# jsdjayanga/kmer-counter

Measured on NVIDIA B200. Metric: k-mers counted/s at k=31, higher is better.
Workload: dtype u64

## Files before the change

### kmer-counter_b200/csrc/kc_super.cu

```cuda
#include <math.h>
#include <stdlib.h>

#include "kc_internal.h"
#include "kc_super.cuh"

namespace kc {

namespace {

constexpr uint32_t kNoBin = 0xffffffffu;
constexpr int kSwThreads = 256;
constexpr int kSwMaxSeg = 18;
constexpr int kNb1Max = 1024;
constexpr int kRsBins = 2048;

template <uint32_t X> struct ILog2 { static constexpr uint32_t v = 1 + ILog2<(X >> 1)>::v; };
template <> struct ILog2<1> { static constexpr uint32_t v = 0; };

__host__ __device__ __forceinline__ uint32_t mmer_hash(uint32_t mm) {
    uint32_t h = mm * 0x9E3779B1u;
    h ^= h >> 15;
    h *= 0x85EBCA6Bu;
    return h;
}
// ... 1003 lines not shown
    if (total) owner = (uint32_t)((bk_lo + (bk_hi - bk_lo) / 2) * P / total);
    if (owner >= P) owner = P - 1;
    atomicMin(&s_lo[owner], bk0);
    __syncthreads();
    if (tid == 0) {
        s_lo[P] = NB;
        for (int o = (int)P - 1; o >= 0; o--)
            if (s_lo[o] > s_lo[o + 1]) s_lo[o] = s_lo[o + 1];
        s_lo[0] = 0;
        if (keep_ranges)
            for (uint32_t o = 0; o <= P; o++) s_lo[o] = x->lo[o];
        for (uint32_t o = 0; o <= P; o++) x->lo[o] = s_lo[o];
        uint32_t widest = 1;
        for (uint32_t o = 0; o < P; o++) {
            const uint32_t wd = ((s_lo[o + 1] + (1u << fold) - 1) >> fold) - (s_lo[o] >> fold);
            widest = wd > widest ? wd : widest;
        }
        while (s_b2 > 0 && ((unsigned long long)widest << s_b2) > kSuperMaxSub) s_b2--;
        s_large = (large_plan || (total >> (b1 + s_b2)) > sub_target) ? 1 : 0;
    }
    __syncthreads();
    const uint32_t my_lo = s_lo[rank], my_hi = s_lo[rank + 1];
    unsigned long long n_recv = 0;
    for (uint32_t s2 = 0; s2 < P; s2++) {
        const unsigned long long incl = block_incl(all_hist[s2 * NB + tid]);
        if (tid == 0) { s_b = 0; s_e = 0; }
        __syncthreads();
        if (my_lo > 0 && tid == (int)my_lo - 1) s_b = incl;
        if (my_hi > 0 && tid == (int)my_hi - 1) s_e = incl;
        __syncthreads();
        if (tid == 0) { x->src_range[s2][0] = (uint32_t)s_b; x->src_range[s2][1] = (uint32_t)s_e; }
        n_recv += s_e - s_b;
        __syncthreads();
    }
    {
        const uint32_t nb1 = 1u << b1;
        uint32_t c = 0;
        if ((uint32_t)tid < nb1)
            for (int j = 0; j < (1 << fold); j++) c += all_hist[rank * NB + ((uint32_t)tid << fold) + j];
        const unsigned long long incl = block_incl(c);
        if ((uint32_t)tid < nb1) {
            base1[tid] = (uint32_t)(incl - c);
            cursor1[tid] = (uint32_t)(incl - c);
            if ((uint32_t)tid == nb1 - 1) base1[nb1] = (uint32_t)incl;
        }
    }
    if (tid == 0) {
        const int b2 = s_b2;
        unsigned long long nd = sc[SW_D];
        if (nd > d_cap) nd = d_cap;
        uint32_t any_ovf = 0;
        for (uint32_t s2 = 0; s2 < P; s2++)
            if (peers.sc[s2][SW_OVF] != 0) any_ovf = 1;
        plan->n_d = (uint32_t)nd;
        plan->b1 = (uint32_t)b1;
        plan->b2 = (uint32_t)b2;
        plan->shift2 = 64 - b1 - b2;
        plan->sub0 = (my_lo >> fold) << b2;
        plan->n_sub = (((my_hi + (1u << fold) - 1) >> fold) << b2) - plan->sub0;
        plan->prefix_bits = b1 + b2;
        x->n_recv = (uint32_t)(n_recv > 0xffffffffull ? 0xffffffffull : n_recv);
        x->any_ovf = any_ovf;
        x->fin_large = (uint32_t)s_large;
        if (n_recv > d_cap) atomicOr(&sc[SW_FAIL], 16ull);
    }
}

struct XPeers {
    const uint64_t *keys[8];
    const uint32_t *counts[8];
    const uint32_t *hist2[8];
};
__global__ void __launch_bounds__(256) x_merge_hist_kernel(XPeers peers, uint32_t P, const SuperPlanDev *__restrict__ plan,
                                                           uint32_t *__restrict__ out) {
    const uint32_t n = plan->n_sub, sub0 = plan->sub0;
    for (uint32_t j = blockIdx.x * blockDim.x + threadIdx.x; j < n; j += gridDim.x * blockDim.x) {
        uint32_t c = 0;
        for (uint32_t s2 = 0; s2 < P; s2++) c += peers.hist2[s2][sub0 + j];
        out[j] = c;
    }
}

constexpr int kRsThreads = 256;
template <int W> struct RsCfg { static constexpr int ITEMS = 16 / W, TILE = kRsThreads * ITEMS; };

template <int W, int LEVEL>
__global__ void __launch_bounds__(kRsThreads) rec_scatter_kernel(const uint64_t *__restrict__ in_keys,
                                                                 const uint32_t *__restrict__ in_counts,
                                                                 uint64_t *__restrict__ out_keys,
                                                                 uint32_t *__restrict__ out_counts,
                                                                 const SuperPlanDev *__restrict__ plan, int b1,
                                                                 const unsigned long long *__restrict__ n_ptr, uint64_t cap,
                                                                 uint32_t *__restrict__ g_cursor,
                                                                 const uint32_t *__restrict__ range) {
    constexpr int ITEMS = RsCfg<W>::ITEMS, TILE = RsCfg<W>::TILE;
    extern __shared__ __align__(16) uint8_t rs_smem[];
    Key<W> *stg_k = reinterpret_cast<Key<W> *>(rs_smem);
    uint32_t *stg_c = reinterpret_cast<uint32_t *>(stg_k + TILE);
    uint32_t *cnt = stg_c + TILE, *start = cnt + kRsBinsPadded, *gbase = start + kRsBinsPadded;
    __shared__ uint32_t s_warp[kRsThreads / 32];
    uint32_t n, first = 0;
    if (LEVEL == 1) {
        unsigned long long nn = *n_ptr;
        n = (uint32_t)(nn > cap ? cap : nn);
    } else if (range) {
        first = range[0];
        n = range[1];
    } else {
        n = plan->n_d;
    }
    const int b2 = LEVEL == 1 ? 0 : (int)plan->b2;
    if (LEVEL == 1) b1 = (int)plan->b1;
    const int shift = LEVEL == 1 ? 64 - b1 : (int)plan->shift2;
    const uint32_t nb2 = 1u << b2;
    const uint32_t sub0 = LEVEL == 1 ? 0u : plan->sub0;
    for (uint32_t begin = first + blockIdx.x * (uint32_t)TILE; begin < n; begin += gridDim.x * (uint32_t)TILE) {
        const uint32_t end = begin + TILE < n ? begin + TILE : n;
        Key<W> key[ITEMS];
        uint32_t val[ITEMS];
        uint16_t rank[ITEMS];
#pragma unroll
        for (int i = 0; i < ITEMS; i++) {
            const uint32_t idx = begin + i * kRsThreads + threadIdx.x;
            if (idx < end) { key[i] = ld_key<W>(in_keys, idx); val[i] = in_counts[idx]; }
            else { key[i].w[0] = 0; val[i] = 0; }
        }
        uint32_t p0 = 0, nb;
        if (LEVEL == 1) {
            nb = 1u << b1;
        } else {
            p0 = ((uint32_t)(in_keys[(size_t)begin * W] >> shift) >> b2) << b2;
            const uint32_t pl = (uint32_t)(in_keys[(size_t)(end - 1) * W] >> shift);
            nb = (pl >> b2) == (p0 >> b2) || 2 * nb2 > (uint32_t)kRsBins ? nb2 : 2 * nb2;
        }
        for (uint32_t i = threadIdx.x; i < nb; i += kRsThreads) cnt[pad32(i)] = 0;
        __syncthreads();
#pragma unroll
        for (int i = 0; i < ITEMS; i++) {
            const uint32_t idx = begin + i * kRsThreads + threadIdx.x;
            rank[i] = 0xffffu;
            if (idx < end) {
                const uint32_t pfx = (uint32_t)(key[i].w[0] >> shift);
                const uint32_t rel = pfx - p0;
                if (rel < nb) rank[i] = (uint16_t)atomicAdd(&cnt[pad32(rel)], 1u);
                else {
                    const uint32_t o = atomicAdd(&g_cursor[pfx - sub0], 1u);
                    st_key<W>(out_keys, o, key[i]);
                    out_counts[o] = val[i];
                }
            }
        }
        __syncthreads();
        const uint32_t total = block_scan_bins<kRsThreads>(cnt, start, (int)nb, s_warp);
        uint32_t reserved[kRsBins / kRsThreads];
#pragma unroll
        for (int u = 0; u < kRsBins / kRsThreads; u++) {
            const uint32_t b = u * kRsThreads + threadIdx.x;
            reserved[u] = 0;
            if (b < nb) {
                const uint32_t c = cnt[pad32(b)];
                if (c) reserved[u] = atomicAdd(&g_cursor[p0 - sub0 + b], c);
            }
        }
#pragma unroll
        for (int i = 0; i < ITEMS; i++)
            if (rank[i] != 0xffffu) {
                const uint32_t o = start[pad32((uint32_t)(key[i].w[0] >> shift) - p0)] + rank[i];
                stg_k[o] = key[i];
                stg_c[o] = val[i];
            }
#pragma unroll
        for (int u = 0; u < kRsBins / kRsThreads; u++) {
            const uint32_t b = u * kRsThreads + threadIdx.x;
            if (b < nb) gbase[pad32(b)] = reserved[u] - start[pad32(b)];
        }
        __syncthreads();
        for (uint32_t i = threadIdx.x; i < total; i += kRsThreads) {
            const Key<W> k = stg_k[i];
            const uint32_t o = gbase[pad32((uint32_t)(k.w[0] >> shift) - p0)] + i;
            st_key<W>(out_keys, o, k);
            out_counts[o] = stg_c[i];
        }
        __syncthreads();
    }
}

template <int W>
__global__ void __launch_bounds__(256) place_init_kernel(const uint64_t *__restrict__ keys, uint32_t *__restrict__ counts,
                                                         uint64_t n, int shift1, uint32_t *__restrict__ hist1,
                                                         unsigned long long *__restrict__ sc) {
    __shared__ uint32_t sh[kNb1Max];
    for (uint32_t i = threadIdx.x; i < kNb1Max; i += 256) sh[i] = 0;
    __syncthreads();
    for (uint64_t i = blockIdx.x * 256ull + threadIdx.x; i < n; i += gridDim.x * 256ull) {
        counts[i] = 1u;
        atomicAdd(&sh[(uint32_t)(keys[i * W] >> shift1)], 1u);
    }
    __syncthreads();
    for (uint32_t i = threadIdx.x; i < kNb1Max; i += 256) {
        const uint32_t c = sh[i];
        if (c) atomicAdd(&hist1[i], c);
    }
    if (blockIdx.x == 0 && threadIdx.x == 0) sc[SW_D] = n;
}

template <int W>
__global__ void place_fix_zero_kernel(const uint64_t *__restrict__ keys, uint32_t *__restrict__ counts,
                                      const unsigned long long *__restrict__ n_invalid) {
    bool zero = true;
    for (int w = 0; w < W; w++) zero = zero && keys[w] == 0;
    if (zero) counts[0] -= (uint32_t)*n_invalid;
}

constexpr uint32_t kH2Chunk = 16384;
template <int W>
__global__ void __launch_bounds__(256) rec_hist2_kernel(const uint64_t *__restrict__ keys,
                                                        const SuperPlanDev *__restrict__ plan,
                                                        uint32_t *__restrict__ g_hist2) {
    __shared__ uint32_t sh[kRsBins];
    const uint32_t n = plan->n_d;
    const int b2 = (int)plan->b2, shift2 = (int)plan->shift2;
    const uint32_t nb2 = 1u << b2, m2 = nb2 - 1;
    for (uint32_t begin = blockIdx.x * kH2Chunk; begin < n; begin += gridDim.x * kH2Chunk) {
        const uint32_t end = begin + kH2Chunk < n ? begin + kH2Chunk : n;
        for (uint32_t i = threadIdx.x; i < nb2; i += 256) sh[i] = 0;
        const uint32_t b0 = (uint32_t)(keys[(size_t)begin * W] >> shift2) >> b2;
        __syncthreads();
#pragma unroll 4
        for (uint32_t i = begin + threadIdx.x; i < end; i += 256) {
            const uint32_t pfx = (uint32_t)(keys[(size_t)i * W] >> shift2);
            if ((pfx >> b2) == b0) atomicAdd(&sh[pfx & m2], 1u);
            else atomicAdd(&g_hist2[pfx], 1u);
        }
        __syncthreads();
        for (uint32_t i = threadIdx.x; i < nb2; i += 256) {
            const uint32_t c = sh[i];
            if (c) atomicAdd(&g_hist2[(size_t)b0 * nb2 + i], c);
        }
        __syncthreads();
    }
}

constexpr uint32_t kScanTile = 4096;
__global__ void __launch_bounds__(1024) sw_scan_kernel(const uint32_t *__restrict__ hist, const uint32_t *__restrict__ n_ptr,
                                                       uint32_t n_host, uint32_t *__restrict__ base,
                                                       uint32_t *__restrict__ cursor, unsigned long long *total_out) {
    __shared__ uint32_t s_w[32];
    __shared__ uint32_t s_carry;
    const uint32_t n = n_ptr ? *n_ptr : n_host;
    const uint32_t tid = threadIdx.x, lane = tid & 31, warp = tid >> 5;
    const uint32_t t0 = blockIdx.x * kScanTile;
    if (t0 >= n) return;
    uint32_t acc = 0;
#pragma unroll 8
    for (uint32_t i = tid; i < t0; i += 1024) acc += hist[i];
#pragma unroll
    for (int o = 16; o > 0; o >>= 1) acc += __shfl_xor_sync(0xffffffffu, acc, o);
    if (lane == 0) s_w[warp] = acc;
    __syncthreads();
    if (tid == 0) {
        uint32_t c = 0;
        for (int w = 0; w < 32; w++) c += s_w[w];
        s_carry = c;
    }
    __syncthreads();
    const uint32_t i0 = t0 + tid * 4;
    uint32_t v[4];
#pragma unroll
    for (int u = 0; u < 4; u++) v[u] = i0 + u < n ? hist[i0 + u] : 0;
    const uint32_t sum = v[0] + v[1] + v[2] + v[3];
    uint32_t incl = sum;
#pragma unroll
    for (int o = 1; o < 32; o <<= 1) {
        uint32_t t = __shfl_up_sync(0xffffffffu, incl, o);
        if (lane >= (uint32_t)o) incl += t;
    }
    __syncthreads();
    if (lane == 31) s_w[warp] = incl;
    __syncthreads();
    uint32_t off = s_carry, tot = 0;
#pragma unroll
    for (uint32_t w = 0; w < 32; w++) {
        const uint32_t x = s_w[w];
        if (w < warp) off += x;
        tot += x;
    }
    uint32_t run = off + incl - sum;
#pragma unroll
    for (int u = 0; u < 4; u++) {
        if (i0 + u < n) { base[i0 + u] = run; if (cursor) cursor[i0 + u] = run; }
        run += v[u];
    }
    if (tid == 0 && t0 + kScanTile >= n) {
        base[n] = s_carry + tot;
        if (total_out) *total_out = s_carry + tot;
    }
}

__device__ __forceinline__ uint32_t pow2_ceil_u32(uint32_t x) { return x <= 1 ? 1u : 1u << (32 - __clz(x - 1)); }

struct FinishParams {
    const uint64_t *in_keys;
    const uint32_t *in_counts;
    const uint32_t *base2;
    const SuperPlanDev *plan;
    uint64_t *out_keys;
    uint32_t *out_counts;
    uint32_t *m_out;
    uint32_t *big;
    unsigned long long *sc;
};

template <int W, int THREADS, int CAP, bool DUP>
__global__ void __launch_bounds__(THREADS) rec_finish_kernel(FinishParams p) {
    constexpr int kPer = CAP / THREADS;
    extern __shared__ __align__(16) uint8_t fs_smem[];
    Key<W> *sk = reinterpret_cast<Key<W> *>(fs_smem);
    Key<W> *fk = sk + (DUP ? CAP : 0);
    uint32_t *scn = reinterpret_cast<uint32_t *>(fk + CAP);
    uint32_t *fc = scn + (DUP ? CAP : 0);
    uint32_t *c3 = fc + CAP;
    uint32_t *s3 = c3 + CAP + CAP / 32;
    __shared__ uint32_t s_maxbin, s_cnt, s_j, s_b, s_e;
    __shared__ uint32_t s_warp[THREADS / 32];
    const uint32_t tid = threadIdx.x, lane = tid & 31, warp = tid >> 5;
    const uint32_t n_sub = p.plan->n_sub;
    const int prefix_bits = (int)p.plan->prefix_bits;
    unsigned long long folded_local = 0;
    uint32_t t1 = 0, t2 = 0, b1 = 0, e1 = 0;
    if (tid == 0) {
        t1 = (uint32_t)atomicAdd(&p.sc[SW_TICKET2], 1ull);
        t2 = t1 < n_sub ? (uint32_t)atomicAdd(&p.sc[SW_TICKET2], 1ull) : n_sub;
        if (t1 < n_sub) { b1 = p.base2[t1]; e1 = p.base2[t1 + 1]; }
    }

    while (true) {
        if (tid == 0) {
            s_j = t1; s_b = b1; s_e = e1;
            t1 = t2;
            if (t1 < n_sub) {
                b1 = p.base2[t1]; e1 = p.base2[t1 + 1];
                t2 = (uint32_t)atomicAdd(&p.sc[SW_TICKET2], 1ull);
            }
        }
        __syncthreads();
        const uint32_t j = s_j;
        if (j >= n_sub) break;
        const uint32_t b = s_b, n = s_e - b;
        if (n == 0) {
            if (tid == 0) { p.big[j] = 0; if (DUP) p.m_out[j] = 0; }
            __syncthreads();
            continue;
        }
        if (n > (uint32_t)CAP) {
            if (tid == 0) {
                p.big[j] = n;
                atomicAdd(&p.sc[SW_BIG], 1ull);
                atomicAdd(&p.sc[SW_BIG_RECORDS], (unsigned long long)n);
                if (DUP) p.m_out[j] = 0;
            }
            __syncthreads();
            continue;
        }
        if (tid == 0) p.big[j] = 0;
        Key<W> rk[kPer];
        uint32_t rc[kPer], rr[kPer];
#pragma unroll
        for (int u = 0; u < kPer; u++) {
            const uint32_t i = u * THREADS + tid;
            if (u * THREADS >= n) break;
            if (i < n) { rk[u] = ld_key<W>(p.in_keys, b + i); rc[u] = p.in_counts[b + i]; }
        }
        uint32_t nb3 = 2 * pow2_ceil_u32(n);
        nb3 = nb3 < 64 ? 64 : (nb3 > (uint32_t)CAP ? (uint32_t)CAP : nb3);
        int shift3 = 64 - prefix_bits - (31 - __clz(nb3));
        if (shift3 < 0) shift3 = 0;
        for (uint32_t i = tid; i < nb3; i += THREADS) c3[pad32(i)] = 0;
        if (tid == 0) { s_maxbin = 0; s_cnt = 0; }
        __syncthreads();
#pragma unroll
        for (int u = 0; u < kPer; u++) {
            const uint32_t i = u * THREADS + tid;
            if (u * THREADS >= n) break;
            if (i < n) rr[u] = atomicAdd(&c3[pad32((uint32_t)(rk[u].w[0] >> shift3) & (nb3 - 1))], 1u);
        }
        __syncthreads();
        {
            const uint32_t per3 = nb3 >= (uint32_t)THREADS ? nb3 / THREADS : 1u;
            const uint32_t b0 = tid * per3;
            uint32_t sum = 0, mx = 0;
            if (b0 < nb3)
                for (uint32_t q = 0; q < per3; q++) { const uint32_t v = c3[pad32(b0 + q)]; sum += v; mx = max(mx, v); }
            if (mx > 2) atomicMax(&s_maxbin, mx);
            uint32_t incl = sum;
#pragma unroll
            for (int o = 1; o < 32; o <<= 1) {
                uint32_t t = __shfl_up_sync(0xffffffffu, incl, o);
// ... 408 lines not shown
cudaError_t super_scatter(const SuperPlan &pl, const void *d_reads, uint64_t n_reads, void *ws,
                          unsigned long long *d_sc, int n_sms, cudaStream_t s) {
    if (pl.W == 1) return super_scatter_w<1>(pl, d_reads, n_reads, ws, d_sc, n_sms, s);
    if (pl.W == 2) return super_scatter_w<2>(pl, d_reads, n_reads, ws, d_sc, n_sms, s);
    return cudaErrorInvalidValue;
}

template <int W, int THREADS, int TSLOTS, int RPT = 2, bool CANON = false>
static cudaError_t launch_count(const SwCountParams &cp, int n_sms, cudaStream_t s) {
    const uint32_t RB = THREADS * RPT, RT = W == 1 ? (RPT > 1 ? RB : 2 * RB) : 1;
    const uint32_t smem = TSLOTS * (8 * W + 4) + RB * 16 * W + THREADS * 4 + kNb1Max * 4 +
                          (THREADS / 32) * (RPT > 1 ? 64 : 96) * (8 * W + 4) + RT * 20 + RB * 4 + 64;
    auto kern = sw_count_kernel<W, THREADS, TSLOTS, RPT, CANON>;
    cudaError_t e = cudaFuncSetAttribute(kern, cudaFuncAttributeMaxDynamicSharedMemorySize, (int)smem);
    if (e != cudaSuccess) return e;
    int per_sm = 1;
    cudaOccupancyMaxActiveBlocksPerMultiprocessor(&per_sm, kern, THREADS, smem);
    if (per_sm < 1) per_sm = 1;
    kern<<<(uint32_t)n_sms * per_sm, THREADS, smem, s>>>(cp);
    return cudaGetLastError();
}

template <int W>
static cudaError_t super_count_bins_w(const SuperPlan &pl, bool add_phantom, void *ws, unsigned long long *d_sc, int n_sms,
                                      cudaStream_t s, void *const *peer_ws = nullptr, uint32_t rank = 0,
                                      uint32_t n_ranks = 1) {
    cudaError_t e;
    SwCountParams cp{};
    const uint32_t n_src = peer_ws ? n_ranks : 1u;
    cp.n_src = n_src;
    for (uint32_t i = 0; i < n_src; i++) {
        void *w = peer_ws ? peer_ws[i] : ws;
        cp.src_cursor[i] = at<uint32_t>(w, pl.off_cursor);
        cp.src_bins[i] = at<uint8_t>(w, pl.off_bins);
        cp.src_sc[i] = peer_ws ? at<unsigned long long>(w, pl.off_sc) : d_sc;
    }
    cp.bin_begin = peer_ws ? (uint32_t)((uint64_t)pl.n_bins * rank / n_ranks) : 0u;
    cp.n_bins = peer_ws ? (uint32_t)((uint64_t)pl.n_bins * (rank + 1) / n_ranks) - cp.bin_begin : pl.n_bins;
    cp.ovf = at<uint8_t>(ws, pl.off_ovf);
    cp.bin_cap = pl.bin_cap; cp.ovf_slice = pl.ovf_slice; cp.ovf_cap = pl.ovf_cap;
    cp.last_mask = pl.last_mask;
    cp.d_keys = at<uint64_t>(ws, pl.off_dk); cp.d_counts = at<uint32_t>(ws, pl.off_dc); cp.d_cap = pl.d_cap;
    cp.hist1 = at<uint32_t>(ws, pl.off_hist1); cp.shift1 = 64 - pl.b1; cp.nb1 = 1 << pl.b1;
    cp.add_phantom = add_phantom ? 1 : 0;
    cp.sc = d_sc;
    if (pl.flags & kPlanCanonical) return W == 1 ? launch_count<1, 512, 4096, 2, true>(cp, n_sms, s)
                                                 : launch_count<2, 512, 4096, 1, true>(cp, n_sms, s);
    static int variant = -1;
    if (variant < 0) { const char *v = getenv("KC_SW_COUNT"); variant = v ? atoi(v) : 0; }
    if constexpr (W == 1) {
        switch (variant) {
            case 1: e = launch_count<1, 256, 2048, 2>(cp, n_sms, s); break;
            case 2: e = launch_count<1, 512, 4096, 1>(cp, n_sms, s); break;
            case 3: e = launch_count<1, 512, 8192, 1>(cp, n_sms, s); break;
            case 4: e = launch_count<1, 128, 4096, 2>(cp, n_sms, s); break;
            case 5: e = launch_count<1, 128, 2048, 2>(cp, n_sms, s); break;
            case 6: e = launch_count<1, 256, 4096, 1>(cp, n_sms, s); break;
            case 7: e = launch_count<1, 256, 4096, 4>(cp, n_sms, s); break;
            case 8: e = launch_count<1, 512, 4096, 1>(cp, n_sms, s); break;
            case 9: e = launch_count<1, 384, 4096, 2>(cp, n_sms, s); break;
            case 10: e = launch_count<1, 256, 4096, 2>(cp, n_sms, s); break;
            default: e = launch_count<1, 512, 4096, 2>(cp, n_sms, s); break;
        }
    } else {
        switch (variant) {
            case 1: e = launch_count<2, 256, 2048, 1>(cp, n_sms, s); break;
            case 2: e = launch_count<2, 256, 4096, 1>(cp, n_sms, s); break;
            case 3: e = launch_count<2, 256, 4096, 2>(cp, n_sms, s); break;
            default: e = launch_count<2, 512, 4096, 1>(cp, n_sms, s); break;
        }
    }
    return e;
}

cudaError_t super_count_bins(const SuperPlan &pl, bool add_phantom, void *ws, unsigned long long *d_sc, int n_sms,
                             cudaStream_t s, void *const *peer_ws, uint32_t rank, uint32_t n_ranks) {
    if (peer_ws && (n_ranks == 0 || n_ranks > 8 || rank >= n_ranks)) return cudaErrorInvalidValue;
    if (pl.W == 1) return super_count_bins_w<1>(pl, add_phantom, ws, d_sc, n_sms, s, peer_ws, rank, n_ranks);
    if (pl.W == 2) return super_count_bins_w<2>(pl, add_phantom, ws, d_sc, n_sms, s, peer_ws, rank, n_ranks);
    return cudaErrorInvalidValue;
}

template <int W>
static cudaError_t super_place_w(const SuperPlan &pl, void *ws, unsigned long long *d_sc, int n_sms, cudaStream_t s,
                                 cudaEvent_t *evs) {
    cudaError_t e;
    uint64_t *dk = at<uint64_t>(ws, pl.off_dk), *ek = ek_of(pl, ws);
    uint32_t *dc = at<uint32_t>(ws, pl.off_dc), *ec = ec_of(pl, ws);
    if (!ek || !ec) return cudaErrorInvalidValue;
    uint32_t *hist1 = at<uint32_t>(ws, pl.off_hist1), *base1 = at<uint32_t>(ws, pl.off_base1),
             *cur1 = at<uint32_t>(ws, pl.off_cur1), *hist2 = at<uint32_t>(ws, pl.off_hist2),
             *base2 = at<uint32_t>(ws, pl.off_base2), *cur2 = at<uint32_t>(ws, pl.off_cur2);
    SuperPlanDev *plan = at<SuperPlanDev>(ws, pl.off_plan);
    const int sig = pl.W == 1 ? 64 - (int)__builtin_ctzll(pl.last_mask ? pl.last_mask : 1) : 64;
    sw_plan_kernel<<<1, 1024, 0, s>>>(hist1, pl.b1, pl.d_cap, pl.sub_target, sig, base1, cur1, plan, d_sc);
    const uint32_t rs_smem = RsCfg<W>::TILE * (8 * W + 4) + 3 * kRsBinsPadded * 4;
    auto k1 = rec_scatter_kernel<W, 1>;
    auto k2 = rec_scatter_kernel<W, 2>;
    if ((e = cudaFuncSetAttribute(k1, cudaFuncAttributeMaxDynamicSharedMemorySize, (int)rs_smem)) != cudaSuccess) return e;
    if ((e = cudaFuncSetAttribute(k2, cudaFuncAttributeMaxDynamicSharedMemorySize, (int)rs_smem)) != cudaSuccess) return e;
    int per_sm = 1;
    cudaOccupancyMaxActiveBlocksPerMultiprocessor(&per_sm, k1, kRsThreads, rs_smem);
    if (per_sm < 1) per_sm = 1;
    const uint32_t grid = (uint32_t)n_sms * per_sm;
    k1<<<grid, kRsThreads, rs_smem, s>>>(dk, dc, ek, ec, plan, pl.b1, &d_sc[SW_D], pl.d_cap, cur1, nullptr);
    if ((e = cudaGetLastError()) != cudaSuccess) return e;
    if (evs) cudaEventRecord(evs[0], s);
    rec_hist2_kernel<W><<<(uint32_t)n_sms * 8, 256, 0, s>>>(ek, plan, hist2);
    sw_scan_kernel<<<(kSuperMaxSub + kScanTile - 1) / kScanTile, 1024, 0, s>>>(hist2, &plan->n_sub, 0, base2, cur2, nullptr);
    if ((e = cudaGetLastError()) != cudaSuccess) return e;
    if (evs) cudaEventRecord(evs[1], s);
    k2<<<grid, kRsThreads, rs_smem, s>>>(ek, ec, dk, dc, plan, pl.b1, &d_sc[SW_D], pl.d_cap, cur2, nullptr);
    if ((e = cudaGetLastError()) != cudaSuccess) return e;
    if (evs) cudaEventRecord(evs[2], s);
    return cudaSuccess;
}

cudaError_t super_place(const SuperPlan &pl, void *ws, unsigned long long *d_sc, int n_sms, cudaStream_t s, cudaEvent_t *evs) {
    if (pl.W == 1) return super_place_w<1>(pl, ws, d_sc, n_sms, s, evs);
    if (pl.W == 2) return super_place_w<2>(pl, ws, d_sc, n_sms, s, evs);
    if (pl.W == 3) return super_place_w<3>(pl, ws, d_sc, n_sms, s, evs);
    if (pl.W == 4) return super_place_w<4>(pl, ws, d_sc, n_sms, s, evs);
    return cudaErrorInvalidValue;
}

cudaError_t place_init(const SuperPlan &pl, void *ws, unsigned long long *d_sc, uint64_t n, int n_sms, cudaStream_t s) {
    cudaError_t e;
    if (n > pl.d_cap) return cudaErrorInvalidValue;
    if ((e = cudaMemsetAsync(ws, 0, pl.off_base1, s)) != cudaSuccess) return e;
    const uint64_t *dk = at<uint64_t>(ws, pl.off_dk);
    uint32_t *dc = at<uint32_t>(ws, pl.off_dc), *hist1 = at<uint32_t>(ws, pl.off_hist1);
    const uint32_t grid = (uint32_t)n_sms * 8;
    const int shift1 = 64 - pl.b1;
    switch (pl.W) {
        case 1: place_init_kernel<1><<<grid, 256, 0, s>>>(dk, dc, n, shift1, hist1, d_sc); break;
        case 2: place_init_kernel<2><<<grid, 256, 0, s>>>(dk, dc, n, shift1, hist1, d_sc); break;
        case 3: place_init_kernel<3><<<grid, 256, 0, s>>>(dk, dc, n, shift1, hist1, d_sc); break;
        case 4: place_init_kernel<4><<<grid, 256, 0, s>>>(dk, dc, n, shift1, hist1, d_sc); break;
        default: return cudaErrorInvalidValue;
    }
    return cudaGetLastError();
}

uint64_t *place_keys(const SuperPlan &pl, void *ws) { return at<uint64_t>(ws, pl.off_dk); }

cudaError_t place_fix_zero(int W, const uint64_t *run_keys, uint32_t *run_counts, const unsigned long long *d_n_invalid,
                           cudaStream_t s) {
    switch (W) {
        case 1: place_fix_zero_kernel<1><<<1, 1, 0, s>>>(run_keys, run_counts, d_n_invalid); break;
        case 2: place_fix_zero_kernel<2><<<1, 1, 0, s>>>(run_keys, run_counts, d_n_invalid); break;
        case 3: place_fix_zero_kernel<3><<<1, 1, 0, s>>>(run_keys, run_counts, d_n_invalid); break;
        case 4: place_fix_zero_kernel<4><<<1, 1, 0, s>>>(run_keys, run_counts, d_n_invalid); break;
        default: return cudaErrorInvalidValue;
    }
    return cudaGetLastError();
}

cudaError_t super_count(const SuperPlan &pl, bool add_phantom, void *ws, unsigned long long *d_sc, int n_sms,
                        cudaStream_t s, cudaEvent_t *evs) {
    cudaError_t e = super_count_bins(pl, add_phantom, ws, d_sc, n_sms, s);
    if (e != cudaSuccess) return e;
    if (evs) cudaEventRecord(evs[0], s);
    return super_place(pl, ws, d_sc, n_sms, s, evs ? evs + 1 : nullptr);
}

void super_tmp_buffers(const SuperPlan &pl, void *ws, uint64_t **tmp_keys, uint32_t **tmp_counts) {
    *tmp_keys = ek_of(pl, ws);
    *tmp_counts = ec_of(pl, ws);
}

template <int W, bool DUP, int THREADS, int CAP>
static cudaError_t super_finish_w(const SuperPlan &pl, void *ws, unsigned long long *d_sc, uint64_t *out_keys,
                                  uint32_t *out_counts, int n_sms, cudaStream_t s) {
    FinishParams fp{};
    fp.in_keys = at<uint64_t>(ws, pl.off_dk);
    fp.in_counts = at<uint32_t>(ws, pl.off_dc);
    fp.base2 = at<uint32_t>(ws, pl.off_base2);
    fp.plan = at<SuperPlanDev>(ws, pl.off_plan);
    fp.out_keys = out_keys;
    fp.out_counts = out_counts;
    fp.m_out = at<uint32_t>(ws, pl.off_mout);
    fp.big = at<uint32_t>(ws, pl.off_big);
    fp.sc = d_sc;
    const uint32_t smem = (DUP ? 2 : 1) * CAP * (8 * W + 4) + 2 * (CAP + CAP / 32) * 4;
    auto kern = rec_finish_kernel<W, THREADS, CAP, DUP>;
    cudaError_t e = cudaFuncSetAttribute(kern, cudaFuncAttributeMaxDynamicSharedMemorySize, (int)smem);
    if (e != cudaSuccess) return e;
    int per_sm = 1;
    cudaOccupancyMaxActiveBlocksPerMultiprocessor(&per_sm, kern, THREADS, smem);
    if (per_sm < 1) per_sm = 1;
    kern<<<(uint32_t)n_sms * per_sm, THREADS, smem, s>>>(fp);
    return cudaGetLastError();
}

template <int W>
static cudaError_t super_finish_d(const SuperPlan &pl, bool dup, void *ws, unsigned long long *d_sc, uint64_t *out_keys,
                                  uint32_t *out_counts, int n_sms, cudaStream_t s) {
    if (pl.fin_cap == kFinCapLarge)
        return dup ? super_finish_w<W, true, 512, kFinCapLarge>(pl, ws, d_sc, out_keys, out_counts, n_sms, s)
                   : super_finish_w<W, false, 512, kFinCapLarge>(pl, ws, d_sc, out_keys, out_counts, n_sms, s);
    return dup ? super_finish_w<W, true, 256, kFinCapSmall>(pl, ws, d_sc, out_keys, out_counts, n_sms, s)
               : super_finish_w<W, false, 256, kFinCapSmall>(pl, ws, d_sc, out_keys, out_counts, n_sms, s);
}

cudaError_t super_finish(const SuperPlan &pl, bool dup, void *ws, unsigned long long *d_sc, uint64_t *out_keys,
                         uint32_t *out_counts, int n_sms, cudaStream_t s) {
    if (pl.W == 1) return super_finish_d<1>(pl, dup, ws, d_sc, out_keys, out_counts, n_sms, s);
    if (pl.W == 2) return super_finish_d<2>(pl, dup, ws, d_sc, out_keys, out_counts, n_sms, s);
    if (!dup || (pl.fin_cap != kFinCapSmall && pl.fin_cap != kFinCapWide)) return cudaErrorInvalidValue;
    if (pl.fin_cap == kFinCapWide) {
        if (pl.W == 3) return super_finish_w<3, true, 256, kFinCapWide>(pl, ws, d_sc, out_keys, out_counts, n_sms, s);
        if (pl.W == 4) return super_finish_w<4, true, 256, kFinCapWide>(pl, ws, d_sc, out_keys, out_counts, n_sms, s);
    } else {
        if (pl.W == 3) return super_finish_w<3, true, 512, kFinCapSmall>(pl, ws, d_sc, out_keys, out_counts, n_sms, s);
        if (pl.W == 4) return super_finish_w<4, true, 512, kFinCapSmall>(pl, ws, d_sc, out_keys, out_counts, n_sms, s);
    }
    return cudaErrorInvalidValue;
}

cudaError_t super_big_gather(const SuperPlan &pl, void *ws, uint64_t *tk, uint32_t *tc, int n_sms, cudaStream_t s) {
    SuperPlanDev *plan = at<SuperPlanDev>(ws, pl.off_plan);
    uint32_t *big = at<uint32_t>(ws, pl.off_big), *bigoff = at<uint32_t>(ws, pl.off_bigoff), *base2 = at<uint32_t>(ws, pl.off_base2);
    sw_scan_kernel<<<(kSuperMaxSub + kScanTile - 1) / kScanTile, 1024, 0, s>>>(big, &plan->n_sub, 0, bigoff, nullptr, nullptr);
    const uint64_t *dk = at<uint64_t>(ws, pl.off_dk);
    const uint32_t *dc = at<uint32_t>(ws, pl.off_dc);
    if (pl.W == 1) big_gather_kernel<1><<<(uint32_t)n_sms * 8, 256, 0, s>>>(dk, dc, base2, big, bigoff, plan, tk, tc);
    else if (pl.W == 2) big_gather_kernel<2><<<(uint32_t)n_sms * 8, 256, 0, s>>>(dk, dc, base2, big, bigoff, plan, tk, tc);
    else if (pl.W == 3) big_gather_kernel<3><<<(uint32_t)n_sms * 8, 256, 0, s>>>(dk, dc, base2, big, bigoff, plan, tk, tc);
    else big_gather_kernel<4><<<(uint32_t)n_sms * 8, 256, 0, s>>>(dk, dc, base2, big, bigoff, plan, tk, tc);
    return cudaGetLastError();
}

cudaError_t super_big_place(const SuperPlan &pl, bool dup, void *ws, unsigned long long *d_sc, const uint64_t *sk,
                            const uint32_t *sc_counts, uint64_t *out_keys, uint32_t *out_counts, int n_sms, cudaStream_t s) {
    const SuperPlanDev *plan = at<SuperPlanDev>(ws, pl.off_plan);
    const uint32_t *big = at<uint32_t>(ws, pl.off_big), *bigoff = at<uint32_t>(ws, pl.off_bigoff), *base2 = at<uint32_t>(ws, pl.off_base2);
    uint32_t *m_out = at<uint32_t>(ws, pl.off_mout);
    const uint32_t grid = (uint32_t)n_sms * 8;
    if (pl.W == 1) {
        if (dup) big_place_kernel<1, true><<<grid, 256, 0, s>>>(sk, sc_counts, base2, big, bigoff, plan, out_keys, out_counts, m_out, d_sc);
        else big_place_kernel<1, false><<<grid, 256, 0, s>>>(sk, sc_counts, base2, big, bigoff, plan, out_keys, out_counts, m_out, d_sc);
    } else if (pl.W == 2) {
        if (dup) big_place_kernel<2, true><<<grid, 256, 0, s>>>(sk, sc_counts, base2, big, bigoff, plan, out_keys, out_counts, m_out, d_sc);
        else big_place_kernel<2, false><<<grid, 256, 0, s>>>(sk, sc_counts, base2, big, bigoff, plan, out_keys, out_counts, m_out, d_sc);
    } else if (pl.W == 3 && dup) {
        big_place_kernel<3, true><<<grid, 256, 0, s>>>(sk, sc_counts, base2, big, bigoff, plan, out_keys, out_counts, m_out, d_sc);
    } else if (pl.W == 4 && dup) {
        big_place_kernel<4, true><<<grid, 256, 0, s>>>(sk, sc_counts, base2, big, bigoff, plan, out_keys, out_counts, m_out, d_sc);
    } else {
        return cudaErrorInvalidValue;
    }
    return cudaGetLastError();
}

cudaError_t super_fold_offsets(const SuperPlan &pl, void *ws, unsigned long long *d_sc, cudaStream_t s) {
    SuperPlanDev *plan = at<SuperPlanDev>(ws, pl.off_plan);
    sw_scan_kernel<<<(kSuperMaxSub + kScanTile - 1) / kScanTile, 1024, 0, s>>>(
        at<uint32_t>(ws, pl.off_mout), &plan->n_sub, 0, at<uint32_t>(ws, pl.off_off), nullptr, &d_sc[SW_OUT]);
    return cudaGetLastError();
}

cudaError_t super_gather(const SuperPlan &pl, void *ws, const uint64_t *tmp_keys, const uint32_t *tmp_counts,
                         uint64_t *out_keys, uint32_t *out_counts, int n_sms, cudaStream_t s) {
    const SuperPlanDev *plan = at<SuperPlanDev>(ws, pl.off_plan);
    const uint32_t *src = at<uint32_t>(ws, pl.off_base2), *off = at<uint32_t>(ws, pl.off_off);
    if (pl.W == 1) sw_gather_kernel<1><<<(uint32_t)n_sms * 8, 256, 0, s>>>(tmp_keys, tmp_counts, src, off, plan, out_keys, out_counts);
    else if (pl.W == 2) sw_gather_kernel<2><<<(uint32_t)n_sms * 8, 256, 0, s>>>(tmp_keys, tmp_counts, src, off, plan, out_keys, out_counts);
    else if (pl.W == 3) sw_gather_kernel<3><<<(uint32_t)n_sms * 8, 256, 0, s>>>(tmp_keys, tmp_counts, src, off, plan, out_keys, out_counts);
    else sw_gather_kernel<4><<<(uint32_t)n_sms * 8, 256, 0, s>>>(tmp_keys, tmp_counts, src, off, plan, out_keys, out_counts);
    return cudaGetLastError();
}

bool super_supported(const SuperPlan &pl) { return super_scatter_fits(pl); }

void super_use_large_finish(SuperPlan *pl) { pl->fin_cap = kFinCapLarge; }

template <int W>
static cudaError_t super_x_local_w(const SuperPlan &pl, void *ws, unsigned long long *d_sc, const uint32_t *d_all_hist,
                                   uint32_t rank, uint32_t n_ranks, bool keep_ranges, void *const *peer_ws, int n_sms,
                                   cudaStream_t s) {
    cudaError_t e;
    if (pl.ext_e) return cudaErrorInvalidValue;
    uint64_t *dk = at<uint64_t>(ws, pl.off_dk), *ek = at<uint64_t>(ws, pl.off_ek);
    uint32_t *dc = at<uint32_t>(ws, pl.off_dc), *ec = at<uint32_t>(ws, pl.off_ec);
    SuperPlanDev *plan = at<SuperPlanDev>(ws, pl.off_plan);
    const int sig = pl.W == 1 ? 64 - (int)__builtin_ctzll(pl.last_mask ? pl.last_mask : 1) : 64;
    XScalars xs{};
    for (uint32_t i = 0; i < n_ranks; i++) xs.sc[i] = peer_ws ? at<unsigned long long>(peer_ws[i], pl.off_sc) : d_sc;
    x_plan_kernel<<<1, 1024, 0, s>>>(d_all_hist, rank, n_ranks, keep_ranges ? 1 : 0, pl.d_cap, pl.sub_target,
                                     pl.fin_cap == kFinCapLarge ? 1 : 0, sig, at<uint32_t>(ws, pl.off_base1),
                                     at<uint32_t>(ws, pl.off_cur1), plan, at<XDev>(ws, pl.off_x), d_sc, xs);
    const uint32_t rs_smem = RsCfg<W>::TILE * (8 * W + 4) + 3 * kRsBinsPadded * 4;
    auto k1 = rec_scatter_kernel<W, 1>;
    if ((e = cudaFuncSetAttribute(k1, cudaFuncAttributeMaxDynamicSharedMemorySize, (int)rs_smem)) != cudaSuccess) return e;
    int per_sm = 1;
    cudaOccupancyMaxActiveBlocksPerMultiprocessor(&per_sm, k1, kRsThreads, rs_smem);
    if (per_sm < 1) per_sm = 1;
    k1<<<(uint32_t)n_sms * per_sm, kRsThreads, rs_smem, s>>>(dk, dc, ek, ec, plan, pl.b1, &d_sc[SW_D], pl.d_cap,
                                                            at<uint32_t>(ws, pl.off_cur1), nullptr);
    rec_hist2_kernel<W><<<(uint32_t)n_sms * 8, 256, 0, s>>>(ek, plan, at<uint32_t>(ws, pl.off_hist2));
    return cudaGetLastError();
}

cudaError_t super_x_local(const SuperPlan &pl, void *ws, unsigned long long *d_sc, const uint32_t *d_all_hist,
                          uint32_t rank, uint32_t n_ranks, bool keep_ranges, void *const *peer_ws, int n_sms, cudaStream_t s) {
    if (pl.b1 != kXB1 || n_ranks == 0 || n_ranks > 8 || rank >= n_ranks) return cudaErrorInvalidValue;
    if (pl.W == 1) return super_x_local_w<1>(pl, ws, d_sc, d_all_hist, rank, n_ranks, keep_ranges, peer_ws, n_sms, s);
    if (pl.W == 2) return super_x_local_w<2>(pl, ws, d_sc, d_all_hist, rank, n_ranks, keep_ranges, peer_ws, n_sms, s);
    return cudaErrorInvalidValue;
}

template <int W>
static cudaError_t super_x_pull_w(const SuperPlan &pl, void *ws, unsigned long long *d_sc, void *const *peer_ws,
                                  uint32_t rank, uint32_t n_ranks, int n_sms, cudaStream_t s) {
    cudaError_t e;
    SuperPlanDev *plan = at<SuperPlanDev>(ws, pl.off_plan);
    XDev *x = at<XDev>(ws, pl.off_x);
    XPeers peers{};
    for (uint32_t i = 0; i < n_ranks; i++) {
        peers.keys[i] = at<uint64_t>(peer_ws[i], pl.off_ek);
        peers.counts[i] = at<uint32_t>(peer_ws[i], pl.off_ec);
        peers.hist2[i] = at<uint32_t>(peer_ws[i], pl.off_hist2);
    }
    uint32_t *h2m = at<uint32_t>(ws, pl.off_h2m), *base2 = at<uint32_t>(ws, pl.off_base2), *cur2 = at<uint32_t>(ws, pl.off_cur2);
    x_merge_hist_kernel<<<(uint32_t)n_sms * 4, 256, 0, s>>>(peers, n_ranks, plan, h2m);
    sw_scan_kernel<<<(kSuperMaxSub + kScanTile - 1) / kScanTile, 1024, 0, s>>>(h2m, &plan->n_sub, 0, base2, cur2, nullptr);
    const uint32_t rs_smem = RsCfg<W>::TILE * (8 * W + 4) + 3 * kRsBinsPadded * 4;
    auto k2 = rec_scatter_kernel<W, 2>;
    if ((e = cudaFuncSetAttribute(k2, cudaFuncAttributeMaxDynamicSharedMemorySize, (int)rs_smem)) != cudaSuccess) return e;
    int per_sm = 1;
    cudaOccupancyMaxActiveBlocksPerMultiprocessor(&per_sm, k2, kRsThreads, rs_smem);
    if (per_sm < 1) per_sm = 1;
    for (uint32_t j = 1; j <= n_ranks; j++) {
        const uint32_t i = (rank + j) % n_ranks;
        k2<<<(uint32_t)n_sms * per_sm, kRsThreads, rs_smem, s>>>(peers.keys[i], peers.counts[i], at<uint64_t>(ws, pl.off_dk),
                                                                at<uint32_t>(ws, pl.off_dc), plan, pl.b1, &d_sc[SW_D],
                                                                pl.d_cap, cur2, &x->src_range[i][0]);
    }
    return cudaGetLastError();
}

cudaError_t super_x_pull(const SuperPlan &pl, void *ws, unsigned long long *d_sc, void *const *peer_ws, uint32_t rank,
                         uint32_t n_ranks, int n_sms, cudaStream_t s) {
    if (n_ranks == 0 || n_ranks > 8 || rank >= n_ranks) return cudaErrorInvalidValue;
    if (pl.W == 1) return super_x_pull_w<1>(pl, ws, d_sc, peer_ws, rank, n_ranks, n_sms, s);
    if (pl.W == 2) return super_x_pull_w<2>(pl, ws, d_sc, peer_ws, rank, n_ranks, n_sms, s);
    return cudaErrorInvalidValue;
}

uint32_t *super_hist1(const SuperPlan &pl, void *ws) { return at<uint32_t>(ws, pl.off_hist1); }
const SuperXInfo *super_x_info(const SuperPlan &pl, void *ws) { return at<XDev>(ws, pl.off_x); }

}

#ifdef KC_SW_PROFILE
extern "C" int kc_sw_profile_read(unsigned long long *out, int reset) {
    cudaError_t e = cudaMemcpyFromSymbol(out, kc::g_sw_prof, sizeof(kc::g_sw_prof));
    if (e == cudaSuccess && reset) {
        static const unsigned long long zero[kc::SWP_SLOTS] = {};
        e = cudaMemcpyToSymbol(kc::g_sw_prof, zero, sizeof(zero));
    }
    return e == cudaSuccess ? 0 : -1;
}
#endif
```

Measured before the change: 60.44 billion.

## Double-buffer scatter tiles via TMA bulk loads and scatter with a shared-memory permutation

The radix scatter kernel now stages each input tile in shared memory through double-buffered 1D TMA bulk copies tracked by mbarriers, so the next tile's load overlaps processing of the current one. It falls back to cooperative loads when the data is unaligned or comes from a peer. It also replaces register-held keys and staged key copies with a 16-bit permutation array, adds per-W tile sizes, and sets a min-blocks launch bound on the finish kernel. The cost is more shared memory per block, which can lower occupancy, plus extra barrier and synchronisation complexity.

Result: no change. 60.14 billion (median of 6 runs) (-0.5%).

```diff
diff --git a/kmer-counter_b200/csrc/kc_super.cu b/kmer-counter_b200/csrc/kc_super.cu
--- a/kmer-counter_b200/csrc/kc_super.cu
+++ b/kmer-counter_b200/csrc/kc_super.cu
@@ -1109,9 +1109,12 @@
 }
 
 constexpr int kRsThreads = 256;
-template <int W> struct RsCfg { static constexpr int ITEMS = 16 / W, TILE = kRsThreads * ITEMS; };
-
-template <int W, int LEVEL>
+
+template <int W, int TILE>
+constexpr uint32_t rs_smem_bytes() {
+    return 2u * TILE * (8 * W + 4) + 2u * TILE * 2 + 2u * kRsBinsPadded * 4 + 2 * 8;
+}
+template <int W, int LEVEL, int TILE>
 __global__ void __launch_bounds__(kRsThreads) rec_scatter_kernel(const uint64_t *__restrict__ in_keys,
                                                                  const uint32_t *__restrict__ in_counts,
                                                                  uint64_t *__restrict__ out_keys,
@@ -1119,13 +1122,16 @@
                                                                  const SuperPlanDev *__restrict__ plan, int b1,
                                                                  const unsigned long long *__restrict__ n_ptr, uint64_t cap,
                                                                  uint32_t *__restrict__ g_cursor,
-                                                                 const uint32_t *__restrict__ range) {
-    constexpr int ITEMS = RsCfg<W>::ITEMS, TILE = RsCfg<W>::TILE;
+                                                                 const uint32_t *__restrict__ range, bool bulk) {
+    constexpr uint32_t kStage = TILE * (8 * W + 4);
     extern __shared__ __align__(16) uint8_t rs_smem[];
-    Key<W> *stg_k = reinterpret_cast<Key<W> *>(rs_smem);
-    uint32_t *stg_c = reinterpret_cast<uint32_t *>(stg_k + TILE);
-    uint32_t *cnt = stg_c + TILE, *start = cnt + kRsBinsPadded, *gbase = start + kRsBinsPadded;
+    uint16_t *rnk = reinterpret_cast<uint16_t *>(rs_smem + 2 * kStage);
+    uint16_t *perm = rnk + TILE;
+    uint32_t *cnt = reinterpret_cast<uint32_t *>(perm + TILE);
+    uint32_t *start = cnt + kRsBinsPadded;
+    uint64_t *bars = reinterpret_cast<uint64_t *>(start + kRsBinsPadded);
     __shared__ uint32_t s_warp[kRsThreads / 32];
+    const uint32_t tid = threadIdx.x;
     uint32_t n, first = 0;
     if (LEVEL == 1) {
         unsigned long long nn = *n_ptr;
@@ -1141,74 +1147,102 @@
     const int shift = LEVEL == 1 ? 64 - b1 : (int)plan->shift2;
     const uint32_t nb2 = 1u << b2;
     const uint32_t sub0 = LEVEL == 1 ? 0u : plan->sub0;
-    for (uint32_t begin = first + blockIdx.x * (uint32_t)TILE; begin < n; begin += gridDim.x * (uint32_t)TILE) {
-        const uint32_t end = begin + TILE < n ? begin + TILE : n;
-        Key<W> key[ITEMS];
-        uint32_t val[ITEMS];
-        uint16_t rank[ITEMS];
-#pragma unroll
-        for (int i = 0; i < ITEMS; i++) {
-            const uint32_t idx = begin + i * kRsThreads + threadIdx.x;
-            if (idx < end) { key[i] = ld_key<W>(in_keys, idx); val[i] = in_counts[idx]; }
-            else { key[i].w[0] = 0; val[i] = 0; }
-        }
+    const uint32_t stride = gridDim.x * (uint32_t)TILE;
+
+    if (tid == 0) {
+        mbar_init(&bars[0], 1);
+        mbar_init(&bars[1], 1);
+        mbar_fence_init();
+    }
+    __syncthreads();
+    auto by_bulk = [&](uint32_t begin, uint32_t m) { return bulk && ((begin | m) & 3u) == 0; };
+    auto issue_load = [&](uint32_t begin, uint32_t s) {
+        const uint32_t m = n - begin < (uint32_t)TILE ? n - begin : (uint32_t)TILE;
+        uint64_t *dk = reinterpret_cast<uint64_t *>(rs_smem + s * kStage);
+        uint32_t *dc = reinterpret_cast<uint32_t *>(rs_smem + s * kStage + TILE * 8 * W);
+        if (by_bulk(begin, m)) {
+            if (tid == 0) {
+                asm volatile("fence.proxy.async.shared::cta;" ::: "memory");
+                mbar_expect_tx(&bars[s], m * (8 * W + 4));
+                tma_load_1d(dk, in_keys + (size_t)begin * W, m * 8 * W, &bars[s]);
+                tma_load_1d(dc, in_counts + begin, m * 4, &bars[s]);
+            }
+        } else {
+#pragma unroll 4
+            for (uint32_t i = tid; i < m * W; i += kRsThreads) dk[i] = in_keys[(size_t)begin * W + i];
+#pragma unroll 4
+            for (uint32_t i = tid; i < m; i += kRsThreads) dc[i] = in_counts[begin + i];
+        }
+    };
+
+    uint32_t stage = 0, phase_bits = 0;
+    uint32_t begin = first + blockIdx.x * (uint32_t)TILE;
+    if (begin < n) issue_load(begin, 0);
+    for (; begin < n; begin += stride) {
+        if (n - begin > stride) issue_load(begin + stride, stage ^ 1);
+        const uint32_t m = n - begin < (uint32_t)TILE ? n - begin : (uint32_t)TILE;
+        if (by_bulk(begin, m)) {
+            mbar_wait(&bars[stage], (phase_bits >> stage) & 1u);
+            phase_bits ^= 1u << stage;
+        } else {
+            __syncthreads();
+        }
+        const uint64_t *sk = reinterpret_cast<const uint64_t *>(rs_smem + stage * kStage);
+        const uint32_t *sc = reinterpret_cast<const uint32_t *>(rs_smem + stage * kStage + TILE * 8 * W);
         uint32_t p0 = 0, nb;
         if (LEVEL == 1) {
             nb = 1u << b1;
         } else {
-            p0 = ((uint32_t)(in_keys[(size_t)begin * W] >> shift) >> b2) << b2;
-            const uint32_t pl = (uint32_t)(in_keys[(size_t)(end - 1) * W] >> shift);
+            p0 = ((uint32_t)(sk[0] >> shift) >> b2) << b2;
+            const uint32_t pl = (uint32_t)(sk[(m - 1) * W] >> shift);
             nb = (pl >> b2) == (p0 >> b2) || 2 * nb2 > (uint32_t)kRsBins ? nb2 : 2 * nb2;
         }
-        for (uint32_t i = threadIdx.x; i < nb; i += kRsThreads) cnt[pad32(i)] = 0;
-        __syncthreads();
-#pragma unroll
-        for (int i = 0; i < ITEMS; i++) {
-            const uint32_t idx = begin + i * kRsThreads + threadIdx.x;
-            rank[i] = 0xffffu;
-            if (idx < end) {
-                const uint32_t pfx = (uint32_t)(key[i].w[0] >> shift);
-                const uint32_t rel = pfx - p0;
-                if (rel < nb) rank[i] = (uint16_t)atomicAdd(&cnt[pad32(rel)], 1u);
-                else {
-                    const uint32_t o = atomicAdd(&g_cursor[pfx - sub0], 1u);
-                    st_key<W>(out_keys, o, key[i]);
-                    out_counts[o] = val[i];
-                }
-            }
+        for (uint32_t i = tid; i < nb; i += kRsThreads) cnt[pad32(i)] = 0;
+        __syncthreads();
+        for (uint32_t i = tid; i < m; i += kRsThreads) {
+            const uint32_t pfx = (uint32_t)(sk[i * W] >> shift);
+            const uint32_t rel = pfx - p0;
+            uint32_t r = 0xffffu;
+            if (rel < nb) {
+                r = atomicAdd(&cnt[pad32(rel)], 1u);
+            } else {
+                const uint32_t o = atomicAdd(&g_cursor[pfx - sub0], 1u);
+                st_key<W>(out_keys, o, ld_key<W>(sk, i));
+                out_counts[o] = sc[i];
+            }
+            rnk[i] = (uint16_t)r;
         }
         __syncthreads();
         const uint32_t total = block_scan_bins<kRsThreads>(cnt, start, (int)nb, s_warp);
         uint32_t reserved[kRsBins / kRsThreads];
 #pragma unroll
         for (int u = 0; u < kRsBins / kRsThreads; u++) {
-            const uint32_t b = u * kRsThreads + threadIdx.x;
+            const uint32_t b = u * kRsThreads + tid;
             reserved[u] = 0;
             if (b < nb) {
                 const uint32_t c = cnt[pad32(b)];
                 if (c) reserved[u] = atomicAdd(&g_cursor[p0 - sub0 + b], c);
             }
         }
-#pragma unroll
-        for (int i = 0; i < ITEMS; i++)
-            if (rank[i] != 0xffffu) {
-                const uint32_t o = start[pad32((uint32_t)(key[i].w[0] >> shift) - p0)] + rank[i];
-                stg_k[o] = key[i];
-                stg_c[o] = val[i];
-            }
+        for (uint32_t i = tid; i < m; i += kRsThreads) {
+            const uint32_t r = rnk[i];
+            if (r != 0xffffu) perm[start[pad32((uint32_t)(sk[i * W] >> shift) - p0)] + r] = (uint16_t)i;
+        }
 #pragma unroll
         for (int u = 0; u < kRsBins / kRsThreads; u++) {
-            const uint32_t b = u * kRsThreads + threadIdx.x;
-            if (b < nb) gbase[pad32(b)] = reserved[u] - start[pad32(b)];
-        }
-        __syncthreads();
-        for (uint32_t i = threadIdx.x; i < total; i += kRsThreads) {
-            const Key<W> k = stg_k[i];
-            const uint32_t o = gbase[pad32((uint32_t)(k.w[0] >> shift) - p0)] + i;
-            st_key<W>(out_keys, o, k);
-            out_counts[o] = stg_c[i];
-        }
-        __syncthreads();
+            const uint32_t b = u * kRsThreads + tid;
+            if (b < nb) cnt[pad32(b)] = reserved[u] - start[pad32(b)];
+        }
+        __syncthreads();
+        for (uint32_t o = tid; o < total; o += kRsThreads) {
+            const uint32_t i = perm[o];
+            const Key<W> k = ld_key<W>(sk, i);
+            const uint32_t g = cnt[pad32((uint32_t)(k.w[0] >> shift) - p0)] + o;
+            st_key<W>(out_keys, g, k);
+            out_counts[g] = sc[i];
+        }
+        __syncthreads();
+        stage ^= 1;
     }
 }
 
@@ -1338,8 +1372,12 @@
     unsigned long long *sc;
 };
 
+template <int W, int CAP, bool DUP>
+constexpr uint32_t fin_smem_bytes() { return (DUP ? 2 : 1) * CAP * (8 * W + 4) + 2 * (CAP + CAP / 32) * 4; }
+template <int W, int CAP, bool DUP>
+constexpr int fin_ctas_per_sm() { return (int)(228u * 1024 / (fin_smem_bytes<W, CAP, DUP>() + 1024 + 256)); }
 template <int W, int THREADS, int CAP, bool DUP>
-__global__ void __launch_bounds__(THREADS) rec_finish_kernel(FinishParams p) {
+__global__ void __launch_bounds__(THREADS, fin_ctas_per_sm<W, CAP, DUP>()) rec_finish_kernel(FinishParams p) {
     constexpr int kPer = CAP / THREADS;
     extern __shared__ __align__(16) uint8_t fs_smem[];
     Key<W> *sk = reinterpret_cast<Key<W> *>(fs_smem);
@@ -1914,6 +1952,29 @@
 }
 
 template <int W>
+constexpr int rs_tile() {
+    return W == 1 ? 3072 : W == 2 ? 2048 : W == 3 ? 1536 : 1024;
+}
+template <int W, int LEVEL>
+static cudaError_t launch_rec_scatter(const uint64_t *in_keys, const uint32_t *in_counts, uint64_t *out_keys,
+                                      uint32_t *out_counts, const SuperPlanDev *plan, int b1,
+                                      const unsigned long long *n_ptr, uint64_t cap, uint32_t *cursor,
+                                      const uint32_t *range, bool bulk, int n_sms, cudaStream_t s) {
+    constexpr int TILE = rs_tile<W>();
+    constexpr uint32_t smem = rs_smem_bytes<W, TILE>();
+    auto kern = rec_scatter_kernel<W, LEVEL, TILE>;
+    bulk = bulk && ((reinterpret_cast<uintptr_t>(in_keys) | reinterpret_cast<uintptr_t>(in_counts)) & 15u) == 0;
+    cudaError_t e = cudaFuncSetAttribute(kern, cudaFuncAttributeMaxDynamicSharedMemorySize, (int)smem);
+    if (e != cudaSuccess) return e;
+    int per_sm = 1;
+    cudaOccupancyMaxActiveBlocksPerMultiprocessor(&per_sm, kern, kRsThreads, smem);
+    if (per_sm < 1) per_sm = 1;
+    kern<<<(uint32_t)n_sms * per_sm, kRsThreads, smem, s>>>(in_keys, in_counts, out_keys, out_counts, plan, b1, n_ptr, cap,
+                                                           cursor, range, bulk);
+    return cudaGetLastError();
+}
+
+template <int W>
 static cudaError_t super_place_w(const SuperPlan &pl, void *ws, unsigned long long *d_sc, int n_sms, cudaStream_t s,
                                  cudaEvent_t *evs) {
     cudaError_t e;
@@ -1926,24 +1987,17 @@
     SuperPlanDev *plan = at<SuperPlanDev>(ws, pl.off_plan);
     const int sig = pl.W == 1 ? 64 - (int)__builtin_ctzll(pl.last_mask ? pl.last_mask : 1) : 64;
     sw_plan_kernel<<<1, 1024, 0, s>>>(hist1, pl.b1, pl.d_cap, pl.sub_target, sig, base1, cur1, plan, d_sc);
-    const uint32_t rs_smem = RsCfg<W>::TILE * (8 * W + 4) + 3 * kRsBinsPadded * 4;
-    auto k1 = rec_scatter_kernel<W, 1>;
-    auto k2 = rec_scatter_kernel<W, 2>;
-    if ((e = cudaFuncSetAttribute(k1, cudaFuncAttributeMaxDynamicSharedMemorySize, (int)rs_smem)) != cudaSuccess) return e;
-    if ((e = cudaFuncSetAttribute(k2, cudaFuncAttributeMaxDynamicSharedMemorySize, (int)rs_smem)) != cudaSuccess) return e;
-    int per_sm = 1;
-    cudaOccupancyMaxActiveBlocksPerMultiprocessor(&per_sm, k1, kRsThreads, rs_smem);
-    if (per_sm < 1) per_sm = 1;
-    const uint32_t grid = (uint32_t)n_sms * per_sm;
-    k1<<<grid, kRsThreads, rs_smem, s>>>(dk, dc, ek, ec, plan, pl.b1, &d_sc[SW_D], pl.d_cap, cur1, nullptr);
-    if ((e = cudaGetLastError()) != cudaSuccess) return e;
+    if ((e = launch_rec_scatter<W, 1>(dk, dc, ek, ec, plan, pl.b1, &d_sc[SW_D], pl.d_cap, cur1, nullptr, true, n_sms, s)) !=
+        cudaSuccess)
+        return e;
     if (evs) cudaEventRecord(evs[0], s);
     rec_hist2_kernel<W><<<(uint32_t)n_sms * 8, 256, 0, s>>>(ek, plan, hist2);
     sw_scan_kernel<<<(kSuperMaxSub + kScanTile - 1) / kScanTile, 1024, 0, s>>>(hist2, &plan->n_sub, 0, base2, cur2, nullptr);
     if ((e = cudaGetLastError()) != cudaSuccess) return e;
     if (evs) cudaEventRecord(evs[1], s);
-    k2<<<grid, kRsThreads, rs_smem, s>>>(ek, ec, dk, dc, plan, pl.b1, &d_sc[SW_D], pl.d_cap, cur2, nullptr);
-    if ((e = cudaGetLastError()) != cudaSuccess) return e;
+    if ((e = launch_rec_scatter<W, 2>(ek, ec, dk, dc, plan, pl.b1, &d_sc[SW_D], pl.d_cap, cur2, nullptr, true, n_sms, s)) !=
+        cudaSuccess)
+        return e;
     if (evs) cudaEventRecord(evs[2], s);
     return cudaSuccess;
 }
@@ -2014,7 +2068,7 @@
     fp.m_out = at<uint32_t>(ws, pl.off_mout);
     fp.big = at<uint32_t>(ws, pl.off_big);
     fp.sc = d_sc;
-    const uint32_t smem = (DUP ? 2 : 1) * CAP * (8 * W + 4) + 2 * (CAP + CAP / 32) * 4;
+    const uint32_t smem = fin_smem_bytes<W, CAP, DUP>();
     auto kern = rec_finish_kernel<W, THREADS, CAP, DUP>;
     cudaError_t e = cudaFuncSetAttribute(kern, cudaFuncAttributeMaxDynamicSharedMemorySize, (int)smem);
     if (e != cudaSuccess) return e;
@@ -2122,14 +2176,9 @@
     x_plan_kernel<<<1, 1024, 0, s>>>(d_all_hist, rank, n_ranks, keep_ranges ? 1 : 0, pl.d_cap, pl.sub_target,
                                      pl.fin_cap == kFinCapLarge ? 1 : 0, sig, at<uint32_t>(ws, pl.off_base1),
                                      at<uint32_t>(ws, pl.off_cur1), plan, at<XDev>(ws, pl.off_x), d_sc, xs);
-    const uint32_t rs_smem = RsCfg<W>::TILE * (8 * W + 4) + 3 * kRsBinsPadded * 4;
-    auto k1 = rec_scatter_kernel<W, 1>;
-    if ((e = cudaFuncSetAttribute(k1, cudaFuncAttributeMaxDynamicSharedMemorySize, (int)rs_smem)) != cudaSuccess) return e;
-    int per_sm = 1;
-    cudaOccupancyMaxActiveBlocksPerMultiprocessor(&per_sm, k1, kRsThreads, rs_smem);
-    if (per_sm < 1) per_sm = 1;
-    k1<<<(uint32_t)n_sms * per_sm, kRsThreads, rs_smem, s>>>(dk, dc, ek, ec, plan, pl.b1, &d_sc[SW_D], pl.d_cap,
-                                                            at<uint32_t>(ws, pl.off_cur1), nullptr);
+    if ((e = launch_rec_scatter<W, 1>(dk, dc, ek, ec, plan, pl.b1, &d_sc[SW_D], pl.d_cap, at<uint32_t>(ws, pl.off_cur1),
+                                      nullptr, true, n_sms, s)) != cudaSuccess)
+        return e;
     rec_hist2_kernel<W><<<(uint32_t)n_sms * 8, 256, 0, s>>>(ek, plan, at<uint32_t>(ws, pl.off_hist2));
     return cudaGetLastError();
 }
@@ -2157,19 +2206,14 @@
     uint32_t *h2m = at<uint32_t>(ws, pl.off_h2m), *base2 = at<uint32_t>(ws, pl.off_base2), *cur2 = at<uint32_t>(ws, pl.off_cur2);
     x_merge_hist_kernel<<<(uint32_t)n_sms * 4, 256, 0, s>>>(peers, n_ranks, plan, h2m);
     sw_scan_kernel<<<(kSuperMaxSub + kScanTile - 1) / kScanTile, 1024, 0, s>>>(h2m, &plan->n_sub, 0, base2, cur2, nullptr);
-    const uint32_t rs_smem = RsCfg<W>::TILE * (8 * W + 4) + 3 * kRsBinsPadded * 4;
-    auto k2 = rec_scatter_kernel<W, 2>;
-    if ((e = cudaFuncSetAttribute(k2, cudaFuncAttributeMaxDynamicSharedMemorySize, (int)rs_smem)) != cudaSuccess) return e;
-    int per_sm = 1;
-    cudaOccupancyMaxActiveBlocksPerMultiprocessor(&per_sm, k2, kRsThreads, rs_smem);
-    if (per_sm < 1) per_sm = 1;
     for (uint32_t j = 1; j <= n_ranks; j++) {
         const uint32_t i = (rank + j) % n_ranks;
-        k2<<<(uint32_t)n_sms * per_sm, kRsThreads, rs_smem, s>>>(peers.keys[i], peers.counts[i], at<uint64_t>(ws, pl.off_dk),
-                                                                at<uint32_t>(ws, pl.off_dc), plan, pl.b1, &d_sc[SW_D],
-                                                                pl.d_cap, cur2, &x->src_range[i][0]);
-    }
-    return cudaGetLastError();
+        if ((e = launch_rec_scatter<W, 2>(peers.keys[i], peers.counts[i], at<uint64_t>(ws, pl.off_dk), at<uint32_t>(ws, pl.off_dc),
+                                          plan, pl.b1, &d_sc[SW_D], pl.d_cap, cur2, &x->src_range[i][0], i == rank, n_sms,
+                                          s)) != cudaSuccess)
+            return e;
+    }
+    return cudaSuccess;
 }
 
 cudaError_t super_x_pull(const SuperPlan &pl, void *ws, unsigned long long *d_sc, void *const *peer_ws, uint32_t rank,
```
